# Saltfish-AB/LatentSync

Hardware: AMD Instinct MI355X
Metric: lip-synced frames/sec at 256x256, 16-frame window, 20 DDIM steps (higher is better)
Workload: dtype bf16; 1 GPU; configs[1]: 256x256 x16-frame windows, 20 DDIM steps, guidance 1.0, LatentSync-1.5 UNet + SD-VAE, bf16; 48 independent windows of a clip batched per UNet call; windows_per_rank=240, windows_per_batch=48, frames_per_window=16, global_batch=768, resolution=256, parallelism=dp1 (window sharding, RCCL all-gather of decoded frames)

## Files before the change

include/ls_hip.h:

```cpp
#ifndef LS_HIP_H
#define LS_HIP_H

#include <stddef.h>
#include <stdint.h>

#ifdef __cplusplus
extern "C" {
#endif

#define LS_ABI_VERSION 14

typedef enum {
  LS_OK = 0,
  LS_ERR_INVALID = 1,
  LS_ERR_LAUNCH = 2,
  LS_ERR_WORKSPACE = 3
} ls_status;

enum { LS_ACT_NONE = 0, LS_ACT_GEGLU = 1, LS_ACT_GELU = 2, LS_ACT_SILU = 3 };

typedef struct {
  const uint16_t* x1; const uint16_t* x2;
  int32_t C1, C2;
  int32_t ld1, ld2;
// ... 75 lines not shown
int ls_attention_fp8(const ls_attn_desc* d, void* workspace, size_t workspace_bytes, void* stream);

typedef struct {
  const uint16_t* x;
  int32_t ldx;
  const float* gamma;
  const float* bpe;
  const uint16_t* w;
  uint16_t* o;
  int32_t ldo;
  int32_t C, heads, n_samples, F, S;
  float eps;
} ls_tattn_desc;

int ls_temporal_attention(const ls_tattn_desc* d, void* stream);

typedef struct {
  const void* x;
  const float* ln_rowstats;
  const void* w1;
  const float* b1;
  const void* w2;
  const float* b2;
  void* y;
  int64_t M;
  int32_t ldx, ldy, C, inner;
} ls_ff_desc;

int ls_feedforward(const ls_ff_desc* d, void* stream);

typedef struct {
  const void* o;
  const void* wo;
  const float* bo;
  const void* h1;
  const void* w1;
  const float* b1;
  const void* w2;
  const float* b2;
  const void* wp;
  const float* bp;
  const void* xb;
  void* z;
  float* cs_out;
  int64_t M;
  int32_t ldo, ldh, ldxb, ldz, C, inner;
  float eps;
} ls_ff_chain_desc;

int ls_ff_chain(const ls_ff_chain_desc* d, void* stream);

typedef struct {
  const void* x;
  const float* ln_rowstats;
  const void* wq;
  const float* bq;
  const void* kv;
  const void* wo;
  const float* bo;
  void* y;
  float* stats_out;
  int64_t M;
  int32_t ldx, ldy, ldkv, C, heads, L, hw;
  float eps;
} ls_xattn_desc;

int ls_cross_attention_block(const ls_xattn_desc* d, void* stream);

int ls_small_linear(const float* x, int32_t M, int32_t K, const uint16_t* w, const float* bias, int32_t N,
                    int32_t silu_in, float* y, void* stream);

int ls_timestep_embed(const int32_t* timesteps, const int32_t* step, int32_t B, int32_t dim, int32_t flip,
                      float shift, float* out, void* stream);

int ls_timestep_embed_f32(const float* ts, int32_t B, int32_t dim, int32_t flip, float shift, float* out,
                          void* stream);

int ls_ddim_cfg_step(const uint16_t* eps, int32_t ld_eps, int32_t Bu, int64_t P, float guidance, float* lat,
                     const float* coef, int32_t* step, uint16_t* unet_in, int32_t ld_in, void* stream);

int ls_prep_pixels(const uint8_t* faces, int32_t F, int32_t R, const float* mask, uint16_t* pix, uint16_t* masked,
                   int32_t ld, void* stream);

int ls_vae_sample(const float* moments, int32_t ld_m, const float* eps, int64_t P, float scaling, float shift,
                  uint16_t* dst, int32_t ld_dst, int32_t c_off, void* stream);

int ls_pack_unet_input(const float* lat, const uint16_t* cond, const float* mask, int32_t F, int32_t R, int32_t h,
                       int32_t Bu, uint16_t* unet_in, int32_t ld_in, void* stream);

int ls_scale_latents(const float* lat, int64_t P, float inv_scaling, float shift, uint16_t* z, int32_t ld,
                     void* stream);

int ls_paste_back(const uint16_t* dec, int32_t ld_dec, const uint16_t* pix, int32_t ld_pix, const float* mask,
                  int32_t F, int32_t R, float* out_nchw, uint8_t* out_u8, void* stream);

int ls_add_rows(const uint16_t* x, int64_t rows, int32_t C, int32_t ldx, const float* table, int32_t table_rows,
                uint16_t* y, int32_t ldy, void* stream);

int ls_set_tuning(int32_t key, int32_t value);

int ls_gemm_occupancy(int32_t which);

size_t ls_log_mel_workspace_bytes(int64_t n_samples, int32_t n_mels);
int ls_log_mel(const float* audio, int64_t n_samples, const float* filters, int32_t n_mels, int64_t t_pad,
               uint16_t* out, void* workspace, size_t workspace_bytes, void* stream);

// ... 56 lines not shown
```

latentsync_amd/_lib.py:

```python
import ctypes as C
import os

HERE = os.path.dirname(os.path.abspath(__file__))
LIB_PATH = os.environ.get("LS_HIP_LIB", os.path.join(HERE, "libls_hip.so"))
ABI_VERSION = 14

c_u16p = C.c_void_p
c_vp = C.c_void_p


class ConvDesc(C.Structure):
    _fields_ = [
        ("x1", c_vp), ("x2", c_vp),
        ("C1", C.c_int32), ("C2", C.c_int32),
        ("ld1", C.c_int32), ("ld2", C.c_int32),
        ("n_img", C.c_int32), ("H", C.c_int32), ("W", C.c_int32),
        ("Ho", C.c_int32), ("Wo", C.c_int32),
        ("ksize", C.c_int32), ("stride", C.c_int32), ("pad", C.c_int32), ("upsample", C.c_int32),
        ("aff_scale", c_vp), ("aff_shift", c_vp), ("imgs_per_sample", C.c_int32), ("silu_in", C.c_int32),
        ("w", c_vp), ("K", C.c_int32), ("N", C.c_int32),
        ("bias", c_vp),
        ("rowvec", c_vp), ("rows_per_vec", C.c_int32), ("rowvec_ld", C.c_int32),
        ("res", c_vp), ("ldr", C.c_int32), ("out_scale", C.c_float),
        ("act", C.c_int32),
        ("y", c_vp), ("ldy", C.c_int32), ("y_f32", C.c_int32),
        ("split_k", C.c_int32),
        ("workspace", c_vp), ("workspace_bytes", C.c_size_t),
        ("ln_rowstats", c_vp), ("ln_colsum", c_vp), ("rowvec_mod", C.c_int32),
        ("row_stats_out", c_vp), ("row_stats_eps", C.c_float),
        ("gn_colsum_out", c_vp),
    ]


class ConvPlanInfo(C.Structure):
    _fields_ = [(f, C.c_int32) for f in (
        "family", "bm", "bn", "ks", "tapu", "buf", "epi", "split", "rb_kt", "rb_fm", "rb_flags",
        "halo_bn", "halo_th", "halo_gn", "halo_cs", "halo_ph", "grid", "threads", "lds_bytes",
        "reduce", "colsum_rows", "row_stats")] + [("workspace_bytes", C.c_int64)]


class AttnDesc(C.Structure):
    _fields_ = [("q", c_vp), ("k", c_vp), ("v", c_vp), ("o", c_vp)] + [
        (f"{t}_{s}", C.c_int64) for t in "qkvo" for s in ("sb1", "sb2", "si", "sh")
    ] + [
        ("batch", C.c_int32), ("z2", C.c_int32), ("heads", C.c_int32), ("nq", C.c_int32),
        ("nk", C.c_int32), ("head_dim", C.c_int32), ("scale", C.c_float),
    ]


class TAttnDesc(C.Structure):
    _fields_ = [("x", c_vp), ("ldx", C.c_int32), ("gamma", c_vp), ("bpe", c_vp), ("w", c_vp), ("o", c_vp),
                ("ldo", C.c_int32), ("C", C.c_int32), ("heads", C.c_int32), ("n_samples", C.c_int32),
                ("F", C.c_int32), ("S", C.c_int32), ("eps", C.c_float)]


class FFDesc(C.Structure):
    _fields_ = [("x", c_vp), ("ln_rowstats", c_vp), ("w1", c_vp), ("b1", c_vp), ("w2", c_vp), ("b2", c_vp),
                ("y", c_vp), ("M", C.c_int64), ("ldx", C.c_int32), ("ldy", C.c_int32), ("C", C.c_int32),
                ("inner", C.c_int32)]


class FFChainDesc(C.Structure):
    _fields_ = [("o", c_vp), ("wo", c_vp), ("bo", c_vp), ("h1", c_vp), ("w1", c_vp), ("b1", c_vp), ("w2", c_vp),
                ("b2", c_vp), ("wp", c_vp), ("bp", c_vp), ("xb", c_vp), ("z", c_vp), ("cs_out", c_vp),
                ("M", C.c_int64), ("ldo", C.c_int32), ("ldh", C.c_int32), ("ldxb", C.c_int32), ("ldz", C.c_int32),
                ("C", C.c_int32), ("inner", C.c_int32), ("eps", C.c_float)]


class XAttnDesc(C.Structure):
    _fields_ = [("x", c_vp), ("ln_rowstats", c_vp), ("wq", c_vp), ("bq", c_vp), ("kv", c_vp), ("wo", c_vp),
                ("bo", c_vp), ("y", c_vp), ("stats_out", c_vp), ("M", C.c_int64), ("ldx", C.c_int32),
                ("ldy", C.c_int32), ("ldkv", C.c_int32), ("C", C.c_int32), ("heads", C.c_int32), ("L", C.c_int32),
                ("hw", C.c_int32), ("eps", C.c_float)]


_SIGS = {
    "ls_abi_version": (C.c_int, []),
    "ls_last_error": (C.c_char_p, []),
    "ls_conv2d": (C.c_int, [C.POINTER(ConvDesc), c_vp]),
    "ls_conv_workspace_bytes": (C.c_size_t, [C.POINTER(ConvDesc)]),
    "ls_conv_path": (C.c_int, [C.POINTER(ConvDesc)]),
    "ls_conv_plan": (C.c_int, [C.POINTER(ConvDesc), C.POINTER(ConvPlanInfo)]),
    "ls_groupnorm": (C.c_int, [c_vp, c_vp, C.c_int32, C.c_int32, C.c_int32, C.c_int64, C.c_int32, C.c_float,
                               c_vp, c_vp, c_vp, c_vp, c_vp, C.c_size_t, c_vp]),
    "ls_groupnorm_workspace_bytes": (C.c_size_t, [C.c_int32, C.c_int32]),
    "ls_groupnorm_colsum": (C.c_int, [c_vp, c_vp, C.c_int32, C.c_int32, C.c_int32, C.c_int64, C.c_int32, C.c_float,
                                      c_vp, c_vp, c_vp, c_vp, c_vp]),
    "ls_gn_colsum": (C.c_int, [c_vp, C.c_int64, C.c_int64, C.c_int32, c_vp, c_vp]),
    "ls_groupnorm_apply": (C.c_int, [c_vp, c_vp, C.c_int32, C.c_int32, C.c_int64, C.c_int64, c_vp, c_vp, C.c_int32,
                                     c_vp, c_vp]),
    "ls_layernorm": (C.c_int, [c_vp, C.c_int64, C.c_int64, C.c_int32, C.c_float, c_vp, c_vp, c_vp, C.c_int32, C.c_int32,
                               c_vp, c_vp]),
    "ls_row_stats": (C.c_int, [c_vp, C.c_int64, C.c_int64, C.c_int32, C.c_float, c_vp, c_vp]),
    "ls_attention": (C.c_int, [C.POINTER(AttnDesc), c_vp]),
    "ls_attention_fp8_workspace_bytes": (C.c_size_t, [C.POINTER(AttnDesc)]),
    "ls_attention_fp8": (C.c_int, [C.POINTER(AttnDesc), c_vp, C.c_size_t, c_vp]),
    "ls_temporal_attention": (C.c_int, [C.POINTER(TAttnDesc), c_vp]),
    "ls_feedforward": (C.c_int, [C.POINTER(FFDesc), c_vp]),
    "ls_cross_attention_block": (C.c_int, [C.POINTER(XAttnDesc), c_vp]),
    "ls_ff_chain": (C.c_int, [C.POINTER(FFChainDesc), c_vp]),
    "ls_small_linear": (C.c_int, [c_vp, C.c_int32, C.c_int32, c_vp, c_vp, C.c_int32, C.c_int32, c_vp, c_vp]),
    "ls_timestep_embed": (C.c_int, [c_vp, c_vp, C.c_int32, C.c_int32, C.c_int32, C.c_float, c_vp, c_vp]),
    "ls_timestep_embed_f32": (C.c_int, [c_vp, C.c_int32, C.c_int32, C.c_int32, C.c_float, c_vp, c_vp]),
    "ls_ddim_cfg_step": (C.c_int, [c_vp, C.c_int32, C.c_int32, C.c_int64, C.c_float, c_vp, c_vp, c_vp, c_vp,
                                   C.c_int32, c_vp]),
    "ls_prep_pixels": (C.c_int, [c_vp, C.c_int32, C.c_int32, c_vp, c_vp, c_vp, C.c_int32, c_vp]),
    "ls_vae_sample": (C.c_int, [c_vp, C.c_int32, c_vp, C.c_int64, C.c_float, C.c_float, c_vp, C.c_int32,
                                C.c_int32, c_vp]),
    "ls_pack_unet_input": (C.c_int, [c_vp, c_vp, c_vp, C.c_int32, C.c_int32, C.c_int32, C.c_int32, c_vp,
                                     C.c_int32, c_vp]),
    "ls_scale_latents": (C.c_int, [c_vp, C.c_int64, C.c_float, C.c_float, c_vp, C.c_int32, c_vp]),
    "ls_paste_back": (C.c_int, [c_vp, C.c_int32, c_vp, C.c_int32, c_vp, C.c_int32, C.c_int32, c_vp, c_vp, c_vp]),
    "ls_set_tuning": (C.c_int, [C.c_int32, C.c_int32]),
    "ls_gemm_occupancy": (C.c_int, [C.c_int32]),
    "ls_log_mel_workspace_bytes": (C.c_size_t, [C.c_int64, C.c_int32]),
    "ls_log_mel": (C.c_int, [c_vp, C.c_int64, c_vp, C.c_int32, C.c_int64, c_vp, c_vp, C.c_size_t, c_vp]),
    "ls_resample": (C.c_int, [c_vp, C.c_int64, c_vp, C.c_int32, C.c_int32, C.c_int32, c_vp, C.c_int64, c_vp]),
    "ls_audio_chunks": (C.c_int, [c_vp, C.c_int64, C.c_int32, C.c_int32, C.c_int32, C.c_int32, C.c_double,
                                  C.c_int32, C.c_int32, c_vp, C.c_int32, c_vp]),
    "ls_face_resize_u8": (C.c_int, [c_vp, C.c_int32, C.c_int32, C.c_int32, C.c_int32, C.c_int32, c_vp, c_vp]),
    "ls_resize_faces_u8": (C.c_int, [c_vp, C.c_int32, C.c_int32, C.c_int32, C.c_int32, C.c_int32, c_vp, c_vp]),
    "ls_restore_tables_bytes": (C.c_size_t, [C.c_int32]),
    "ls_restore_init_tables": (C.c_int, [c_vp, C.c_int32, c_vp]),
    "ls_restore_workspace_bytes": (C.c_size_t, [C.c_int32, C.c_int32, C.c_int32]),
    "ls_restore_frames": (C.c_int, [c_vp, C.c_int32, C.c_int32, C.c_int32, c_vp, C.c_int32, C.c_int32, c_vp, c_vp,
                                    C.c_int32, C.c_int32, C.c_int32, c_vp, c_vp, C.c_size_t, c_vp]),
    "ls_resize_lanczos4_workspace_bytes": (C.c_size_t, [C.c_int32, C.c_int32]),
    "ls_resize_lanczos4_u8": (C.c_int, [c_vp, C.c_int32, C.c_int32, C.c_int32, C.c_int32, c_vp, C.c_int32, C.c_int32,
                                        c_vp, C.c_size_t, c_vp]),
    "ls_align_warp_u8": (C.c_int, [c_vp, C.c_int32, C.c_int32, C.c_int32, c_vp, C.c_int32, C.c_int32, C.c_int32,
                                   c_vp, c_vp, c_vp]),
    "ls_mjpeg_restart_interval": (C.c_int, []),
    "ls_mjpeg_workspace_bytes": (C.c_size_t, [C.c_int32, C.c_int32, C.c_int32]),
    "ls_mjpeg_encode": (C.c_int, [c_vp, C.c_int32, C.c_int32, C.c_int32, C.c_int32, c_vp, C.c_int64, c_vp, c_vp,
                                  C.c_size_t, c_vp]),
    "ls_mjpeg_decode_workspace_bytes": (C.c_size_t, [C.c_int32, C.c_int32, C.c_int32]),
    "ls_mjpeg_decode": (C.c_int, [c_vp, C.c_int64, c_vp, C.c_int32, C.c_int32, C.c_int32, c_vp, C.c_int32, c_vp,
                                  C.c_int32, C.c_int32, c_vp, c_vp, c_vp, C.c_size_t, c_vp]),
    "ls_face_brighten_workspace_bytes": (C.c_size_t, [C.c_int32, C.c_int32, C.c_int32, C.c_int32]),
    "ls_face_brighten": (C.c_int, [c_vp, C.c_int32, C.c_int32, C.c_int32, c_vp, c_vp, C.c_int32, C.c_int32, C.c_int32,
                                   C.c_int32, C.c_int32, C.c_int32, c_vp, C.c_int32, C.c_int32, C.c_float, C.c_int32,
                                   C.c_int32, C.c_int32, c_vp, C.c_size_t, c_vp]),
    "ls_add_rows":(C.c_int, [c_vp, C.c_int64, C.c_int32, C.c_int32, c_vp, C.c_int32, c_vp, C.c_int32, c_vp]),
}

EXPORTED = tuple(_SIGS)

_lib = None


def load(path: str = None):
    global _lib
    if _lib is not None:
# ... 22 lines not shown
```

latentsync_amd/build.py:

```python
import concurrent.futures as cf
import os
import re
import shutil
import subprocess
import sys
import tempfile
import warnings

HERE = os.path.dirname(os.path.abspath(__file__))
REPO = os.path.dirname(HERE)
CSRC = os.path.join(HERE, "csrc")
OBJ = os.path.join(REPO, "build", "obj")
LIB = os.path.join(HERE, "libls_hip.so")
HIPCC = os.environ.get("HIPCC", "/opt/rocm/bin/hipcc")
FLAGS = ["--offload-arch=gfx950", "-O3", "-fPIC", "-std=c++17", "-Wno-unused-result", "-munsafe-fp-atomics",
         "-fno-slp-vectorize"]


def _deps():
    hdrs = [os.path.join(CSRC, f) for f in os.listdir(CSRC) if f.endswith(".h")]
    hdrs.append(os.path.join(REPO, "include", "ls_hip.h"))
    return max(os.path.getmtime(h) for h in hdrs)


COUNTED_VMCNT = ("gemm_rowblock_kernel", "conv_gemm_dma_kernel", "attn5_kernel", "attn8_kernel", "tattn_fused_kernel",
                 "attnw_kernel", "conv3x3_halo_kernel", "ff_chain_kernel")


def _spills(stderr):
    bad, cur = [], None
    for line in stderr.splitlines():
        m = re.search(r"remark: +Function Name: (\S+)", line)
        if m:
            cur = m.group(1)
            continue
        m = re.search(r"remark: +VGPRs Spill: (\d+)", line)
        if m and cur and int(m.group(1)) > 0 and any(k in cur for k in COUNTED_VMCNT):
            bad.append(f"{cur}: {line.split('remark:')[1].strip()}")
    return bad


OBJDUMP = os.environ.get("LLVM_OBJDUMP", "/opt/rocm/lib/llvm/bin/llvm-objdump")
_PK_OPSEL = re.compile(r"v_pk_\w+_f32\b[^\n]*\bop_sel:\[([01,]+)\]")


def _packed_opsel(obj):
    skip = os.environ.get("LS_SKIP_OPSEL_GUARD", "") not in ("", "0")
    if not os.path.exists(OBJDUMP):
        if skip:
            warnings.warn(f"packed-fp32 op_sel guard skipped (LS_SKIP_OPSEL_GUARD): {OBJDUMP} not found")
            return []
        raise RuntimeError(f"packed-fp32 op_sel guard: {OBJDUMP} not found (LS_SKIP_OPSEL_GUARD=1 to build without it)")
    with tempfile.TemporaryDirectory() as td:
        cp = os.path.join(td, "k.o")
        shutil.copy(obj, cp)
        r = subprocess.run([OBJDUMP, "--offloading", cp], capture_output=True, text=True, cwd=td)
        dev = [f for f in os.listdir(td) if "gfx950" in f]
        if r.returncode != 0 or not dev:
            msg = f"could not extract the gfx950 code object of {obj} ({r.stderr.strip()[:200]})"
            if skip:
                warnings.warn("packed-fp32 op_sel guard skipped (LS_SKIP_OPSEL_GUARD): " + msg)
                return []
            raise RuntimeError("packed-fp32 op_sel guard: " + msg + " (LS_SKIP_OPSEL_GUARD=1 to build without it)")
        r = subprocess.run([OBJDUMP, "-d", "--mcpu=gfx950", os.path.join(td, dev[0])], capture_output=True, text=True)
    return [m.group(0).split("//")[0].strip() for m in _PK_OPSEL.finditer(r.stdout) if "1" in m.group(1)]


def _compile(src, obj, dep_time):
    if os.path.exists(obj) and os.path.getmtime(obj) >= max(os.path.getmtime(src), dep_time):
        return obj, None
    cmd = [HIPCC] + FLAGS + ["-Rpass-analysis=kernel-resource-usage", "-c", src, "-o", obj]
    r = subprocess.run(cmd, capture_output=True, text=True)
    if r.returncode != 0:
        return obj, r.stderr
    with open(obj[:-2] + ".remarks", "w") as f:
        f.write(r.stderr)
    bad = _spills(r.stderr)
    if bad:
        os.remove(obj)
# ... 38 lines not shown
```

latentsync_amd/ops.py:

```python
import ctypes as C
import math

import torch

from . import _lib
from ._lib import check

ACT_NONE, ACT_GEGLU, ACT_GELU, ACT_SILU = 0, 1, 2, 3
_GN_EPILOGUE = True
GN_SLOT_ROWS = 128
_UPS_PHASE = True


def _p(t):
    return None if t is None else t.data_ptr()


def _stream():
    return torch.cuda.current_stream().cuda_stream


class Workspace:

    def __init__(self, device, gemm_bytes=256 << 20, gn_bytes=24 << 20):
# ... 274 lines not shown
    lib = _lib.load()
    M, C_ = x2d.shape
    if out is None:
        out = torch.empty((M, C_), dtype=torch.bfloat16, device=x2d.device)
    d = _lib.FFDesc()
    d.x, d.ln_rowstats, d.w1, d.b1 = _p(x2d), _p(ln_stats), _p(w1.w), _p(w1.bias)
    d.w2, d.b2, d.y = _p(w2ff), _p(w2.bias), _p(out)
    d.M, d.ldx, d.ldy, d.C, d.inner = M, x2d.stride(0), out.stride(0), C_, w1.N // 2
    check(lib.ls_feedforward(C.byref(d), _stream()), "ls_feedforward")
    return out


class FFChainPack:

    def __init__(self, wo, bo, w1, b1, w2, b2, wp, bp, C, inner, eps):
        self.wo, self.bo, self.w1, self.b1, self.w2, self.b2, self.wp, self.bp = wo, bo, w1, b1, w2, b2, wp, bp
        self.C, self.inner, self.eps = C, inner, eps


def pack_ff_chain(wo: "Packed", ff1: "Packed", ff2: "Packed", po: "Packed", eps=1e-5):
    from .packing import pack_ff_w2, permute_k_acc
    Cc = wo.N
    bf = lambda t: t.to(torch.bfloat16).contiguous()
    w1 = permute_k_acc(ff1.w.float())
    return FFChainPack(bf(pack_ff_w2(wo.w.float()[:, :Cc], permute=False)), wo.bias.float().contiguous(), bf(w1),
                       ff1.bias.float().contiguous(), bf(pack_ff_w2(ff2.w.float()[:, :ff2.K])),
                       ff2.bias.float().contiguous(), bf(pack_ff_w2(po.w.float()[:, :Cc])),
                       po.bias.float().contiguous(), Cc, ff1.N // 2, eps)


def ff_chain_ok(o2d, pk: "FFChainPack"):
    return (pk is not None and o2d.shape[1] == 320 and pk.inner == 1280 and o2d.shape[0] % 128 == 0
            and o2d.stride(1) == 1 and o2d.stride(0) % 8 == 0)


def ff_chain(o2d, h1, xb, pk: "FFChainPack", shape=None, gn_out=True):
    lib = _lib.load()
    M, C_ = o2d.shape
    res = torch.empty(shape or (M, C_), dtype=torch.bfloat16, device=o2d.device)
    out = res.view(M, C_)
    cs = torch.empty((M // GN_SLOT_ROWS, 2, C_), dtype=torch.float32, device=o2d.device) if gn_out else None
    d = _lib.FFChainDesc()
    d.o, d.wo, d.bo, d.h1 = _p(o2d), _p(pk.wo), _p(pk.bo), _p(h1)
    d.w1, d.b1, d.w2, d.b2, d.wp, d.bp = _p(pk.w1), _p(pk.b1), _p(pk.w2), _p(pk.b2), _p(pk.wp), _p(pk.bp)
    d.xb, d.z, d.cs_out = _p(xb), _p(out), _p(cs)
    d.M, d.ldo, d.ldh, d.ldxb, d.ldz = M, o2d.stride(0), h1.stride(0), xb.stride(0), out.stride(0)
    d.C, d.inner, d.eps = C_, pk.inner, float(pk.eps)
    check(lib.ls_ff_chain(C.byref(d), _stream()), "ls_ff_chain")
    if cs is not None:
        res.gn_cs = cs
    return res


class XAttnPack:

    def __init__(self, wq, bq, wo, bo, C, heads):
        self.wq, self.bq, self.wo, self.bo, self.C, self.heads = wq, bq, wo, bo, C, heads


def pack_cross_attention(wq, ln_weight, ln_bias, wo, bo, heads, device):
    from .packing import pack_xattn_q, pack_xattn_wo
    w = wq.float().cpu()
    gamma, beta = ln_weight.float().cpu(), ln_bias.float().cpu()
    pq, pb = pack_xattn_q(w * gamma[None, :], w @ beta, heads)
    po = pack_xattn_wo(wo.float().cpu(), heads)
    bf = lambda t: t.to(torch.bfloat16).to(device).contiguous()
    return XAttnPack(bf(pq), pb.to(device).contiguous(), bf(po), bo.float().to(device).contiguous(), w.shape[0], heads)


def cross_attention_ok(x2d, pk, L, hw):
    return (pk is not None and x2d.shape[1] == 320 and pk.heads == 8 and 1 <= L <= 64 and hw % 128 == 0
            and x2d.shape[0] % hw == 0 and x2d.stride(1) == 1 and x2d.stride(0) % 8 == 0)


def cross_attention_block(x2d, ln_stats, pk: XAttnPack, kv, L, hw, stats_out, out=None, eps=1e-5):
    lib = _lib.load()
    M, C_ = x2d.shape
    if out is None:
        out = torch.empty((M, C_), dtype=torch.bfloat16, device=x2d.device)
    assert stats_out.dtype == torch.float32 and stats_out.is_contiguous() and stats_out.numel() == 2 * M
    assert kv.stride(1) == 1 and kv.shape[0] == (M // hw) * L and kv.shape[1] >= 2 * C_
    d = _lib.XAttnDesc()
    d.x, d.ln_rowstats, d.wq, d.bq, d.kv, d.wo, d.bo = _p(x2d), _p(ln_stats), _p(pk.wq), _p(pk.bq), _p(kv), \
        _p(pk.wo), _p(pk.bo)
    d.y, d.stats_out = _p(out), _p(stats_out)
    d.M, d.ldx, d.ldy, d.ldkv, d.C, d.heads, d.L, d.hw, d.eps = M, x2d.stride(0), out.stride(0), kv.stride(0), C_, \
        pk.heads, L, hw, eps
    check(lib.ls_cross_attention_block(C.byref(d), _stream()), "ls_cross_attention_block")
    return out


def attention_fp8_workspace_bytes(*, batch, heads, nk, head_dim):
    lib = _lib.load()
    d = _lib.AttnDesc()
    d.batch, d.z2, d.heads, d.nq, d.nk, d.head_dim = batch, 1, heads, 1, nk, head_dim
    return lib.ls_attention_fp8_workspace_bytes(C.byref(d))


def small_linear(x, w, bias, silu_in=False, out=None):
    lib = _lib.load()
    M, K = x.shape
    N = w.shape[0]
    if out is None:
        out = torch.empty((M, N), dtype=torch.float32, device=x.device)
    check(lib.ls_small_linear(_p(x), M, K, _p(w), _p(bias), N, int(silu_in), _p(out), _stream()), "ls_small_linear")
    return out
# ... 218 lines not shown
```

latentsync_amd/unet.py:

```python
import math
from dataclasses import dataclass

import torch

from . import ops
from .config import STAGE2_MODEL
from .packing import geglu_interleave, pack_ff_w2, pack_phase_weight, pack_weight, pad_bias
from .schema import unet_param_shapes
from .weights import fill_state_dict

_FUSED_TEMPORAL = True
_FUSED_FF = True
_FF_CHAIN = True
_NARROW_OUT = True
_FUSED_XATTN = False


def _ff(h, st, ff1, ff2, ff2p):
    if ff2p is not None and ops.feedforward_ok(h, ff1, ff2):
        return ops.feedforward(h, st, ff1, ff2, ff2p)
    g = ops.linear(h, ff1, act=ops.ACT_GEGLU, ln_stats=st)
    return ops.linear(g, ff2, res=h)


def _chain_pack(o, ff1, ff2, po, c):
    if not (_FF_CHAIN and _FUSED_FF and c == 320 and ff1.N == 2560 and ff2.N == 320 and ff2.K == 1280):
        return None
    return ops.pack_ff_chain(o, ff1, ff2, po)


def _ff2_packed(dv, key):
    w = dv.sd[key]
    if not _FUSED_FF or tuple(w.shape) != (320, 1280):
        return None
    return pack_ff_w2(w.float().cpu()).to(torch.bfloat16).to(dv.device).contiguous()

_DEFAULTS = dict(
    sample_size=None, in_channels=4, out_channels=4, center_input_sample=False, flip_sin_to_cos=True, freq_shift=0,
    down_block_types=("CrossAttnDownBlock3D", "CrossAttnDownBlock3D", "CrossAttnDownBlock3D", "DownBlock3D"),
    mid_block_type="UNetMidBlock3DCrossAttn",
    up_block_types=("UpBlock3D", "CrossAttnUpBlock3D", "CrossAttnUpBlock3D", "CrossAttnUpBlock3D"),
    only_cross_attention=False, block_out_channels=(320, 640, 1280, 1280), layers_per_block=2, downsample_padding=1,
    mid_block_scale_factor=1, act_fn="silu", norm_num_groups=32, norm_eps=1e-5, cross_attention_dim=1280,
    attention_head_dim=8, dual_cross_attention=False, use_linear_projection=False, class_embed_type=None,
    num_class_embeds=None, upcast_attention=False, resnet_time_scale_shift="default", use_inflated_groupnorm=False,
    use_motion_module=False, motion_module_resolutions=(1, 2, 4, 8), motion_module_mid_block=False,
    motion_module_decoder_only=False, motion_module_type=None, motion_module_kwargs={}, add_audio_layer=False,
)


class FrozenDict(dict):
    def __getattr__(self, k):
        try:
            return self[k]
        except KeyError as e:
            raise AttributeError(k) from e


@dataclass
class UNet3DConditionOutput:
    sample: torch.Tensor

    def __getitem__(self, i):
        return (self.sample,)[i]


def positional_encoding(d_model, max_len=24):
    position = torch.arange(max_len).unsqueeze(1)
# ... 31 lines not shown
            pk.phase = pack_phase_weight(w).to(torch.bfloat16).to(self.device).contiguous()
        return pk

    def packed_ln(self, w, b, ln, geglu=False, pe=None):
        gamma, beta = (t.detach().float().cpu() for t in ln)
        w = w.float().cpu()
        b = (b.float().cpu() if b is not None else torch.zeros(w.shape[0])) + w @ beta
        pk = self.packed(None, w=w * gamma[None, :], b=b, geglu=geglu)
        pk.colsum = pk.w.float().sum(1).contiguous()
        if pe is not None:
            pk.pe_rows = (pe.float().cpu() @ w.T).to(self.device).contiguous()
        return pk


class _Resnet:
    def __init__(self, dv, p, cin, cout, groups, eps, out_scale, temb_slot):
        self.groups, self.eps, self.cin, self.cout = groups, eps, cin, cout
        self.n1 = (dv.f32(p + ".norm1.weight"), dv.f32(p + ".norm1.bias"))
        self.n2 = (dv.f32(p + ".norm2.weight"), dv.f32(p + ".norm2.bias"))
        self.c1 = dv.packed(p + ".conv1.weight", p + ".conv1.bias")
        self.c2 = dv.packed(p + ".conv2.weight", p + ".conv2.bias")
        self.sc = dv.packed(p + ".conv_shortcut.weight", p + ".conv_shortcut.bias") \
            if (p + ".conv_shortcut.weight") in dv.sd else None
        self.out_scale = 1.0 / out_scale
        self.temb_slot = temb_slot

    def __call__(self, x, B, temb_all, x2=None):
        n = x.shape[0]
        F = n // B
        pps = F * x.shape[1] * x.shape[2]
        s1 = ops.group_norm(x, self.groups, self.eps, *self.n1, B, x2=x2)
        rpv = pps * B if temb_all.shape[0] == 1 else pps
        h = ops.conv(x, self.c1, x2=x2, aff=(s1[0], s1[1], F, True), aff_materialize=True,
                     rowvec=(temb_all[:, self.temb_slot:], rpv, temb_all.shape[1]), gn_out=True)
        s2 = ops.group_norm(h, self.groups, self.eps, *self.n2, B)
        res = x if self.sc is None else ops.conv(x, self.sc, x2=x2)
        return ops.conv(h, self.c2, aff=(s2[0], s2[1], F, True), aff_materialize=True, res=res,
                        out_scale=self.out_scale, gn_out=True)


class _Transformer:
    def __init__(self, dv, p, c, heads, groups, audio):
        self.c, self.heads, self.groups = c, heads, groups
        self.fp8 = False
        self.norm = (dv.f32(p + ".norm.weight"), dv.f32(p + ".norm.bias"))
        self.proj_in = dv.packed(p + ".proj_in.weight", p + ".proj_in.bias")
        self.proj_out = dv.packed(p + ".proj_out.weight", p + ".proj_out.bias")
        b = p + ".transformer_blocks.0"
        sd = dv.sd
        ln = lambda k: (sd[k + ".weight"], sd[k + ".bias"])
        self.qkv1 = dv.packed_ln(torch.cat([sd[f"{b}.attn1.to_{n}.weight"] for n in "qkv"], 0), None, ln(b + ".norm1"))
        self.o1 = dv.packed(b + ".attn1.to_out.0.weight", b + ".attn1.to_out.0.bias")
        self.has_audio = audio and (b + ".attn2.to_q.weight") in sd
        if self.has_audio:
            self.q2 = dv.packed_ln(sd[b + ".attn2.to_q.weight"], None, ln(b + ".norm2"))
            self.kv2 = dv.packed(None, w=torch.cat([sd[b + ".attn2.to_k.weight"], sd[b + ".attn2.to_v.weight"]], 0))
            self.o2 = dv.packed(b + ".attn2.to_out.0.weight", b + ".attn2.to_out.0.bias")
            self.xa = ops.pack_cross_attention(
                sd[b + ".attn2.to_q.weight"], *ln(b + ".norm2"), sd[b + ".attn2.to_out.0.weight"],
                sd[b + ".attn2.to_out.0.bias"], heads, dv.device) if _FUSED_XATTN and c == 320 and heads == 8 else None
        self.ff1 = dv.packed_ln(sd[b + ".ff.net.0.proj.weight"], sd[b + ".ff.net.0.proj.bias"], ln(b + ".norm3"),
                                geglu=True)
        self.ff2 = dv.packed(b + ".ff.net.2.weight", b + ".ff.net.2.bias")
        self.ff2p = _ff2_packed(dv, b + ".ff.net.2.weight")
        self.chain = _chain_pack(self.o2, self.ff1, self.ff2, self.proj_out, c) if self.has_audio else None

    def audio_kv(self, audio_rows):
        return ops.linear(audio_rows, self.kv2) if self.has_audio else None

    def __call__(self, x, audio_rows, n_audio_tok, kv=None):
        n, H, W, C = x.shape
        HW = H * W
        rows = n * HW
        d = C // self.heads
        sc = ops.group_norm(x, self.groups, 1e-6, *self.norm, n)
        st = torch.empty((rows, 2), dtype=torch.float32, device=x.device)
        h = ops.conv(x, self.proj_in, aff=(sc[0], sc[1], 1, False), aff_materialize=True,
                     stats_out=st).view(rows, C)
        qkv = ops.linear(h, self.qkv1, ln_stats=st)
        o = torch.empty((rows, C), dtype=torch.bfloat16, device=x.device)
        ops.attention(qkv, qkv[:, C:], qkv[:, 2 * C:], o, batch=n, z2=1, heads=self.heads, nq=HW, nk=HW, head_dim=d,
                      qs=(HW * 3 * C, 0, 3 * C, d), ks=(HW * 3 * C, 0, 3 * C, d), vs=(HW * 3 * C, 0, 3 * C, d),
                      os_=(HW * C, 0, C, d), fp8=self.fp8 and HW > 128 and d in (40, 80))
        h = ops.linear(o, self.o1, res=h, stats_out=st)
        if self.has_audio and audio_rows is not None:
            if kv is None:
                kv = ops.linear(audio_rows, self.kv2)
            L = n_audio_tok
            if ops.cross_attention_ok(h, self.xa, L, HW):
                st2 = torch.empty_like(st)
                h = ops.cross_attention_block(h, st, self.xa, kv, L, HW, st2)
                st = st2
                return self._tail(x, h, st, n, H, W, C)
            q = ops.linear(h, self.q2, ln_stats=st)
            ops.attention(q, kv, kv[:, C:], o, batch=n, z2=1, heads=self.heads, nq=HW, nk=L, head_dim=d,
                          qs=(HW * C, 0, C, d), ks=(L * 2 * C, 0, 2 * C, d), vs=(L * 2 * C, 0, 2 * C, d),
                          os_=(HW * C, 0, C, d))
            if ops.ff_chain_ok(o, self.chain):
                return ops.ff_chain(o, h, x.view(rows, C), self.chain, shape=(n, H, W, C))
            h = ops.linear(o, self.o2, res=h, stats_out=st)
        return self._tail(x, h, st, n, H, W, C)

    def _tail(self, x, h, st, n, H, W, C):
        h = _ff(h, st, self.ff1, self.ff2, self.ff2p)
        return ops.conv(h.view(n, H, W, C), self.proj_out, res=x, gn_out=True)


class _Motion:
    def __init__(self, dv, p, c, heads, groups, kw):
        t = p + ".temporal_transformer"
        b = t + ".transformer_blocks.0"
        sd = dv.sd
        self.c, self.heads, self.groups = c, heads, groups
        self.norm = (dv.f32(t + ".norm.weight"), dv.f32(t + ".norm.bias"))
        self.proj_in = dv.packed(t + ".proj_in.weight", t + ".proj_in.bias")
        self.proj_out = dv.packed(t + ".proj_out.weight", t + ".proj_out.bias")
        self.attn = []
        i = 0
        max_len = kw.get("temporal_position_encoding_max_len", 24)
        while f"{b}.attention_blocks.{i}.to_q.weight" in sd:
            a = f"{b}.attention_blocks.{i}"
            pe = sd.get(a + ".pos_encoder.pe")
            if kw.get("temporal_position_encoding", False):
                pe = (pe.reshape(-1, c) if pe is not None else positional_encoding(c, max_len)).float()
                pe = pe.to(dv.device).contiguous()
            else:
                pe = None
            ln = (sd[f"{b}.norms.{i}.weight"], sd[f"{b}.norms.{i}.bias"])
            wqkv = [sd[f"{a}.to_{n}.weight"] for n in "qkv"]
            self.attn.append(dict(
                qkv=dv.packed_ln(torch.cat(wqkv, 0), None, ln, pe=pe),
                fused=ops.pack_temporal(*wqkv, *ln, pe, heads, dv.device) if c in (320, 640) and heads == 8
                else None,
                o=dv.packed(a + ".to_out.0.weight", a + ".to_out.0.bias")))
            i += 1
        self.ff1 = dv.packed_ln(sd[b + ".ff.net.0.proj.weight"], sd[b + ".ff.net.0.proj.bias"],
                                (sd[b + ".ff_norm.weight"], sd[b + ".ff_norm.bias"]), geglu=True)
        self.ff2 = dv.packed(b + ".ff.net.2.weight", b + ".ff.net.2.bias")
        self.ff2p = _ff2_packed(dv, b + ".ff.net.2.weight")
        self.chain = _chain_pack(self.attn[-1]["o"], self.ff1, self.ff2, self.proj_out, c) if self.attn else None

    def __call__(self, x, B):
        n, H, W, C = x.shape
        F = n // B
        S = H * W
        rows = n * S
        d = C // self.heads
# ... 378 lines not shown
```

Baseline: 158.0 frames/s.

## Fuse back-to-back linears with LayerNorm stats into one chain kernel

Adds a HIP kernel that chains two linears in one launch. The first is either proj_in with the GroupNorm affine applied to the input, or attn1's out-projection with a residual. The kernel computes each row's LayerNorm mean and rstd in-register, normalizes the intermediate, and runs the LN-folded second linear (qkv1 or q2) straight from registers. This removes a kernel launch and the HBM re-read of the intermediate for C=320 transformer blocks. In exchange it is a large hand-tuned kernel with triple-buffered LDS staging, fixed to C=320 and M divisible by 256, and it computes statistics in double.

```diff
diff --git a/include/ls_hip.h b/include/ls_hip.h
--- a/include/ls_hip.h
+++ b/include/ls_hip.h
@@ -151,6 +151,25 @@
 
 typedef struct {
   const void* x;
+  const void* w1;
+  const float* b1;
+  const float* aff_scale;
+  const float* aff_shift;
+  const void* res;
+  const void* w2;
+  const float* b2;
+  void* h;
+  float* stats;
+  void* y;
+  int64_t M, rows_per_sample;
+  int32_t ldx, ldr, ldh, ldy, C, N2;
+  float eps;
+} ls_linear_chain_desc;
+
+int ls_linear_chain(const ls_linear_chain_desc* d, void* stream);
+
+typedef struct {
+  const void* x;
   const float* ln_rowstats;
   const void* wq;
   const float* bq;
diff --git a/latentsync_amd/_lib.py b/latentsync_amd/_lib.py
--- a/latentsync_amd/_lib.py
+++ b/latentsync_amd/_lib.py
@@ -67,6 +67,13 @@
                 ("C", C.c_int32), ("inner", C.c_int32), ("eps", C.c_float)]
 
 
+class LinearChainDesc(C.Structure):
+    _fields_ = [("x", c_vp), ("w1", c_vp), ("b1", c_vp), ("aff_scale", c_vp), ("aff_shift", c_vp), ("res", c_vp),
+                ("w2", c_vp), ("b2", c_vp), ("h", c_vp), ("stats", c_vp), ("y", c_vp), ("M", C.c_int64),
+                ("rows_per_sample", C.c_int64), ("ldx", C.c_int32), ("ldr", C.c_int32), ("ldh", C.c_int32),
+                ("ldy", C.c_int32), ("C", C.c_int32), ("N2", C.c_int32), ("eps", C.c_float)]
+
+
 class XAttnDesc(C.Structure):
     _fields_ = [("x", c_vp), ("ln_rowstats", c_vp), ("wq", c_vp), ("bq", c_vp), ("kv", c_vp), ("wo", c_vp),
                 ("bo", c_vp), ("y", c_vp), ("stats_out", c_vp), ("M", C.c_int64), ("ldx", C.c_int32),
@@ -99,6 +106,7 @@
     "ls_feedforward": (C.c_int, [C.POINTER(FFDesc), c_vp]),
     "ls_cross_attention_block": (C.c_int, [C.POINTER(XAttnDesc), c_vp]),
     "ls_ff_chain": (C.c_int, [C.POINTER(FFChainDesc), c_vp]),
+    "ls_linear_chain": (C.c_int, [C.POINTER(LinearChainDesc), c_vp]),
     "ls_small_linear": (C.c_int, [c_vp, C.c_int32, C.c_int32, c_vp, c_vp, C.c_int32, C.c_int32, c_vp, c_vp]),
     "ls_timestep_embed": (C.c_int, [c_vp, c_vp, C.c_int32, C.c_int32, C.c_int32, C.c_float, c_vp, c_vp]),
     "ls_timestep_embed_f32": (C.c_int, [c_vp, C.c_int32, C.c_int32, C.c_int32, C.c_float, c_vp, c_vp]),
diff --git a/latentsync_amd/build.py b/latentsync_amd/build.py
--- a/latentsync_amd/build.py
+++ b/latentsync_amd/build.py
@@ -24,7 +24,7 @@
 
 
 COUNTED_VMCNT = ("gemm_rowblock_kernel", "conv_gemm_dma_kernel", "attn5_kernel", "attn8_kernel", "tattn_fused_kernel",
-                 "attnw_kernel", "conv3x3_halo_kernel", "ff_chain_kernel")
+                 "attnw_kernel", "conv3x3_halo_kernel", "ff_chain_kernel", "linear_chain_kernel")
 
 
 def _spills(stderr):
diff --git a/latentsync_amd/csrc/ls_chain.hip b/latentsync_amd/csrc/ls_chain.hip
--- /dev/null
+++ b/latentsync_amd/csrc/ls_chain.hip
@@ -0,0 +1,287 @@
+#include "ls_common.h"
+
+namespace ls {
+
+struct ChainArgs {
+  const u16 *x, *w1, *w2, *res;
+  const float *b1, *b2, *aff_scale, *aff_shift;
+  u16 *h, *y;
+  float* stats;
+  int ldx, ldr, ldh, ldy, N2, rps;
+  float eps;
+};
+
+template <int KT, int FM, bool RES>
+__global__ void __launch_bounds__(512) linear_chain_kernel(ChainArgs a) {
+  constexpr int FN = 2, BN = 16 * FN, BM = 8 * 16 * FM, C = 32 * KT;
+  constexpr int KTILES = KT / 2;
+  constexpr int WIMG = BN * KTILES * 8;
+  constexpr int RIMG = RES ? BM * BN / 8 : 0;
+  constexpr int RPT = RIMG / 512;
+  constexpr int STAGE = WIMG + 16 + RIMG;
+  constexpr int PPT = (WIMG + 511) / 512;
+  constexpr int NSTORE = FM * FN;
+  static_assert(KT % 2 == 0 && WIMG % 256 == 0 && RIMG % 512 == 0, "K a multiple of 64");
+  extern __shared__ __attribute__((aligned(16))) uint4 lds_dyn[];
+  const int tid = threadIdx.x, lane = tid & 63, wid = tid >> 6;
+  const int l16 = lane & 15, lg = lane >> 4;
+  const int rb = blockIdx.x;
+  const int mw = rb * BM + wid * 16 * FM;
+  const int nc2 = a.N2 / BN;
+
+  const int wid_u = __builtin_amdgcn_readfirstlane(wid);
+  __builtin_assume(wid_u >= 0 && wid_u < 8);
+  const i32x4 rs_w1 = buffer_rsrc(a.w1, (uint32_t)(C * C * 2));
+  const i32x4 rs_w2 = buffer_rsrc(a.w2, (uint32_t)(a.N2 * C * 2));
+  const i32x4 rs_r = RES ? buffer_rsrc(a.res + (long)rb * BM * a.ldr, (uint32_t)(BM * a.ldr * 2)) : rs_w1;
+  static_assert(8 * BN == 256 && BN / 8 == 4, "piece arithmetic below");
+  int wvo, rvo;
+  {
+    const int t = tid >> 8, row = (tid >> 3) & 31, pc = tid & 7;
+    const int lc = pc ^ ((row >> 1) & 7);
+    wvo = (row * C + t * 64 + lc * 8) * 2;
+    rvo = ((tid >> 2) * a.ldr + (tid & 3) * 8) * 2;
+  }
+  lds_u4* const lbase = (lds_u4*)lds_dyn;
+  auto issue_w = [&](const i32x4& rs, const float* bias, int c, int stage) {
+    lds_u4* const dst = lbase + stage * STAGE;
+#pragma unroll
+    for (int p = 0; p < PPT; ++p) {
+      if (WIMG % 512 == 0 || p * 512 + wid_u * 64 < WIMG)
+        ls_raw_buffer_load_lds(rs, (__attribute__((address_space(3))) void*)(dst + p * 512 + wid_u * 64), 16, wvo,
+                               c * BN * C * 2 + p * 256, 0, 0);
+    }
+    if (wid == 0 && lane < BN / 4) glds16(bias + c * BN + lane * 4, lds_dyn + stage * STAGE + WIMG);
+  };
+  auto issue1 = [&](int c, int stage) {
+    issue_w(rs_w1, a.b1, c, stage);
+    lds_u4* const dst = lbase + stage * STAGE;
+#pragma unroll
+    for (int p = 0; p < RPT; ++p)
+      ls_raw_buffer_load_lds(rs_r, (__attribute__((address_space(3))) void*)(dst + WIMG + 16 + p * 512 + wid_u * 64), 16,
+                             rvo, c * BN * 2 + p * 256 * a.ldr, 0, 0);
+  };
+  auto issue2 = [&](int t, int stage) { issue_w(rs_w2, a.b2, t, stage); };
+
+  issue1(0, 0);
+  bf16x8 ar[FM][KT];
+#pragma unroll
+  for (int i = 0; i < FM; ++i) {
+    const u16* src = a.x + (long)(mw + i * 16 + l16) * a.ldx + lg * 8;
+#pragma unroll
+    for (int s = 0; s < KT; ++s) ar[i][s] = *(const bf16x8*)(src + s * 32);
+  }
+  if (!RES) {
+    const long sb = (long)(mw / a.rps) * C + lg * 8;
+    wait_vm<0>();
+#pragma unroll
+    for (int s = 0; s < KT; ++s) {
+      float sc[8], sh[8];
+      load8f(a.aff_scale + sb + s * 32, sc);
+      load8f(a.aff_shift + sb + s * 32, sh);
+#pragma unroll
+      for (int i = 0; i < FM; ++i) {
+        bf16x8 v = ar[i][s];
+#pragma unroll
+        for (int e = 0; e < 8; ++e) v[e] = (__bf16)fmaf((float)v[e], sc[e], sh[e]);
+        asm volatile("" : "+v"(v));
+        ar[i][s] = v;
+      }
+    }
+  }
+  wait_vm<0>();
+  __builtin_amdgcn_s_barrier();
+  asm volatile("" ::: "memory");
+
+  f32x4 acc[2][FM][FN];
+  bf16x8 op[FM][KT];
+  auto load_prm = [&](int stage, float4 (&bb)[FN]) {
+    const float4* prm = (const float4*)(lds_dyn + stage * STAGE + WIMG);
+#pragma unroll
+    for (int j = 0; j < FN; ++j) bb[j] = prm[lg + 4 * j];
+  };
+  double S1[FM], S2[FM];
+#pragma unroll
+  for (int i = 0; i < FM; ++i) { S1[i] = 0.0; S2[i] = 0.0; }
+  auto epilogue1 = [&](int c, f32x4 (&ac)[FM][FN], int stage) {
+    const int nb = c * BN + 4 * lg;
+    const u16* rtile = (const u16*)(lds_dyn + stage * STAGE + WIMG + 16);
+#pragma unroll
+    for (int i = 0; i < FM; ++i) {
+      u16* hrow = a.h + (long)(mw + i * 16 + l16) * a.ldh;
+      float cs1 = 0.f, cs2 = 0.f;
+      uint2 pk[FN];
+#pragma unroll
+      for (int j = 0; j < FN; ++j) {
+        float r4[4] = {0.f, 0.f, 0.f, 0.f};
+        if (RES) {
+          const uint2 rs = *(const uint2*)(rtile + (wid * 16 * FM + i * 16 + l16) * BN + 4 * lg + 16 * j);
+          r4[0] = __uint_as_float(rs.x << 16); r4[1] = __uint_as_float(rs.x & 0xffff0000u);
+          r4[2] = __uint_as_float(rs.y << 16); r4[3] = __uint_as_float(rs.y & 0xffff0000u);
+        }
+        pk[j] = make_uint2(pack2(ac[i][j][0] + r4[0], ac[i][j][1] + r4[1]), pack2(ac[i][j][2] + r4[2], ac[i][j][3] + r4[3]));
+        *(uint2*)(hrow + nb + 16 * j) = pk[j];
+        typedef __bf16 bf2 __attribute__((ext_vector_type(2)));
+        const bf2 one2 = {(__bf16)1.0f, (__bf16)1.0f};
+        const bf2 px = __builtin_bit_cast(bf2, pk[j].x), py = __builtin_bit_cast(bf2, pk[j].y);
+        cs1 = __builtin_amdgcn_fdot2_f32_bf16(py, one2, __builtin_amdgcn_fdot2_f32_bf16(px, one2, cs1, false), false);
+        cs2 = __builtin_amdgcn_fdot2_f32_bf16(py, py, __builtin_amdgcn_fdot2_f32_bf16(px, px, cs2, false), false);
+      }
+      S1[i] += (double)cs1;
+      S2[i] += (double)cs2;
+      op[i][c] = __builtin_bit_cast(bf16x8, make_uint4(pk[0].x, pk[0].y, pk[1].x, pk[1].y));
+    }
+  };
+  auto epilogue2 = [&](int t, f32x4 (&ac)[FM][FN]) {
+    const int nb = t * BN + 4 * lg;
+#pragma unroll
+    for (int i = 0; i < FM; ++i) {
+      u16* yrow = a.y + (long)(mw + i * 16 + l16) * a.ldy;
+#pragma unroll
+      for (int j = 0; j < FN; ++j)
+        *(uint2*)(yrow + nb + 16 * j) = make_uint2(pack2(ac[i][j][0], ac[i][j][1]), pack2(ac[i][j][2], ac[i][j][3]));
+    }
+  };
+  auto mfma_chunk = [&](const bf16x8 (&b)[FM][KT], int stage, f32x4 (&ac)[FM][FN], const float4 (&b0)[FN]) {
+    const uint4* cur = lds_dyn + stage * STAGE;
+#pragma unroll
+    for (int i = 0; i < FM; ++i)
+#pragma unroll
+      for (int j = 0; j < FN; ++j) ac[i][j] = (f32x4){b0[j].x, b0[j].y, b0[j].z, b0[j].w};
+#pragma unroll
+    for (int s = 0; s < KT; ++s) {
+      bf16x8 bw[FN];
+      const int ch = (s & 1) * 4 + lg;
+#pragma unroll
+      for (int j = 0; j < FN; ++j)
+        bw[j] = __builtin_bit_cast(bf16x8, cur[(s >> 1) * (8 * BN) + swz64(j * 16 + l16, ch)]);
+#pragma unroll
+      for (int i = 0; i < FM; ++i)
+#pragma unroll
+        for (int j = 0; j < FN; ++j)
+          ac[i][j] = __builtin_amdgcn_mfma_f32_16x16x32_bf16(bw[j], b[i][s], ac[i][j], 0, 0, 0);
+    }
+  };
+  auto sync = [&]() {
+    asm volatile("s_waitcnt lgkmcnt(0)" ::: "memory");
+    __builtin_amdgcn_s_barrier();
+    asm volatile("" ::: "memory");
+  };
+
+  {
+    float4 bn[FN];
+    load_prm(0, bn);
+    issue1(1, 1);
+    mfma_chunk(ar, 0, acc[0], bn);
+  }
+  wait_vm<0>();
+  sync();
+#pragma unroll
+  for (int c = 1; c < KT; ++c) {
+    float4 bn[FN];
+    load_prm(c % 3, bn);
+    if (c + 1 < KT) issue1(c + 1, (c + 1) % 3);
+    else issue2(0, (c + 1) % 3);
+    mfma_chunk(ar, c % 3, acc[c & 1], bn);
+    epilogue1(c - 1, acc[(c - 1) & 1], (c - 1) % 3);
+    wait_vm<NSTORE>();
+    sync();
+  }
+  epilogue1(KT - 1, acc[(KT - 1) & 1], (KT - 1) % 3);
+
+#pragma unroll
+  for (int i = 0; i < FM; ++i) {
+    double s1 = S1[i], s2 = S2[i];
+#pragma unroll
+    for (int o = 16; o < 64; o <<= 1) {
+      s1 += __shfl_xor(s1, o, 64);
+      s2 += __shfl_xor(s2, o, 64);
+    }
+    const double n = (double)C, mean = s1 / n;
+    const double var = fmax(s2 / n - mean * mean, 0.0);
+    const float meanf = (float)mean, rstd = (float)(1.0 / sqrt(var + (double)a.eps));
+    if (lg == 0) *(float2*)(a.stats + 2L * (mw + i * 16 + l16)) = make_float2(meanf, rstd);
+    const float nmr = -meanf * rstd;
+#pragma unroll
+    for (int s = 0; s < KT; ++s) {
+      bf16x8 v = op[i][s];
+#pragma unroll
+      for (int e = 0; e < 8; ++e) v[e] = (__bf16)fmaf((float)v[e], rstd, nmr);
+      op[i][s] = v;
+    }
+  }
+
+  {
+    float4 bn[FN];
+    load_prm(KT % 3, bn);
+    issue2(min(1, nc2 - 1), (KT + 1) % 3);
+    mfma_chunk(op, KT % 3, acc[0], bn);
+  }
+  wait_vm<0>();
+  sync();
+  auto body2 = [&](int t, f32x4 (&ac)[FM][FN], f32x4 (&prev)[FM][FN]) {
+    const int st = (KT + t) % 3;
+    float4 bn[FN];
+    load_prm(st, bn);
+    issue2(min(t + 1, nc2 - 1), st == 2 ? 0 : st + 1);
+    mfma_chunk(op, st, ac, bn);
+    epilogue2(t - 1, prev);
+    wait_vm<NSTORE>();
+    sync();
+  };
+  int t = 1;
+  for (; t + 1 < nc2; t += 2) {
+    body2(t, acc[1], acc[0]);
+    body2(t + 1, acc[0], acc[1]);
+  }
+  if (t < nc2) {
+    body2(t, acc[1], acc[0]);
+    epilogue2(t, acc[1]);
+  } else {
+    epilogue2(nc2 - 1, acc[0]);
+  }
+}
+
+template <int KT, int FM, bool RES>
+static int launch_chain(const ChainArgs& a, long M, hipStream_t s) {
+  constexpr int BM = 128 * FM;
+  constexpr size_t shm = (size_t)3 * (32 * (KT / 2) * 8 + 16 + (RES ? BM * 32 / 8 : 0)) * 16;
+  LS_SET_MAX_DYN_SHM((linear_chain_kernel<KT, FM, RES>), (int)shm);
+  linear_chain_kernel<KT, FM, RES><<<(unsigned)(M / BM), 512, shm, s>>>(a);
+  return check_launch("linear_chain_kernel");
+}
+
+}
+
+using namespace ls;
+
+extern "C" int ls_linear_chain(const ls_linear_chain_desc* d, void* stream) {
+  if (!d || !d->x || !d->w1 || !d->b1 || !d->w2 || !d->b2 || !d->h || !d->stats || !d->y)
+    return fail(LS_ERR_INVALID, "ls_linear_chain: null pointer");
+  const bool aff = d->aff_scale || d->aff_shift;
+  if (aff == (d->res != nullptr) || (aff && (!d->aff_scale || !d->aff_shift)))
+    return fail(LS_ERR_INVALID, "ls_linear_chain: either aff_scale + aff_shift (form i) or res (form ii)");
+  if (d->C != 320) return fail(LS_ERR_INVALID, "ls_linear_chain: C = 320 only");
+  if (d->N2 != d->C && d->N2 != 3 * d->C) return fail(LS_ERR_INVALID, "ls_linear_chain: N2 = C or 3 C only");
+  const int bm = 256;
+  if (d->M <= 0 || d->M % bm || d->M > 0x7fffffffL)
+    return fail(LS_ERR_INVALID, "ls_linear_chain: M a positive multiple of 256, < 2^31");
+  const int32_t ldmax = 1 << 20;
+  if (d->ldx < d->C || d->ldh < d->C || d->ldy < d->N2 || d->ldx % 8 || d->ldh % 4 || d->ldy % 4 || d->ldx > ldmax ||
+      d->ldh > ldmax || d->ldy > ldmax || (d->res && (d->ldr < d->C || d->ldr % 8 || d->ldr > ldmax)))
+    return fail(LS_ERR_INVALID, "ls_linear_chain: pitches >= the row length, <= 2^20 (x, res: % 8; h, y: % 4)");
+  if (aff && (d->rows_per_sample <= 0 || d->rows_per_sample > 0x7fffffffL || d->rows_per_sample % (bm / 8)))
+    return fail(LS_ERR_INVALID, "ls_linear_chain: rows_per_sample a positive multiple of 32 (a wave's rows)");
+  if ((((uintptr_t)d->x | (uintptr_t)d->w1 | (uintptr_t)d->w2 | (uintptr_t)d->b1 | (uintptr_t)d->b2 | (uintptr_t)d->res |
+        (uintptr_t)d->aff_scale | (uintptr_t)d->aff_shift) & 15) ||
+      (((uintptr_t)d->h | (uintptr_t)d->y | (uintptr_t)d->stats) & 7))
+    return fail(LS_ERR_INVALID, "ls_linear_chain: x / w1 / w2 / b1 / b2 / res / aff 16-B aligned, h / y / stats 8-B aligned");
+  ChainArgs a;
+  a.x = (const u16*)d->x; a.w1 = (const u16*)d->w1; a.w2 = (const u16*)d->w2; a.res = (const u16*)d->res;
+  a.b1 = d->b1; a.b2 = d->b2; a.aff_scale = d->aff_scale; a.aff_shift = d->aff_shift;
+  a.h = (u16*)d->h; a.y = (u16*)d->y; a.stats = d->stats;
+  a.ldx = d->ldx; a.ldr = d->ldr; a.ldh = d->ldh; a.ldy = d->ldy; a.N2 = d->N2; a.rps = (int)d->rows_per_sample;
+  a.eps = d->eps;
+  hipStream_t s = (hipStream_t)stream;
+  return aff ? launch_chain<10, 2, false>(a, d->M, s) : launch_chain<10, 2, true>(a, d->M, s);
+}
diff --git a/latentsync_amd/ops.py b/latentsync_amd/ops.py
--- a/latentsync_amd/ops.py
+++ b/latentsync_amd/ops.py
@@ -350,6 +350,51 @@
     return res
 
 
+class LinearChainPack:
+
+    def __init__(self, w1, b1, w2, b2, C, N2, eps):
+        self.w1, self.b1, self.w2, self.b2, self.C, self.N2, self.eps = w1, b1, w2, b2, C, N2, eps
+
+
+def pack_linear_chain(first: "Packed", second_ln: "Packed", eps=1e-5):
+    from .packing import permute_k_acc
+    assert second_ln.colsum is not None, "the second linear must be LayerNorm-folded"
+    w2 = permute_k_acc(second_ln.w.float()).to(torch.bfloat16).contiguous()
+    return LinearChainPack(first.w, first.bias, w2, second_ln.bias.float().contiguous(), first.N, second_ln.N, eps)
+
+
+def linear_chain_ok(x2d, pk: "LinearChainPack", *, res=None, rows_per_sample=None):
+    if pk is None or pk.C != 320 or tuple(pk.w1.shape) != (pk.C, pk.C) or pk.N2 not in (pk.C, 3 * pk.C):
+        return False
+    bm = 256
+    if x2d.dim() != 2 or x2d.shape[1] != pk.C or x2d.shape[0] % bm or x2d.stride(1) != 1 or x2d.stride(0) % 8:
+        return False
+    if res is not None:
+        return res.stride(1) == 1 and res.stride(0) % 8 == 0 and res.data_ptr() % 16 == 0
+    return rows_per_sample is not None and rows_per_sample % (bm // 8) == 0
+
+
+def linear_chain(x2d, pk: "LinearChainPack", stats_out, *, aff=None, rows_per_sample=0, res=None, h=None, out=None):
+    lib = _lib.load()
+    M, C_ = x2d.shape
+    if h is None:
+        h = torch.empty((M, C_), dtype=torch.bfloat16, device=x2d.device)
+    if out is None:
+        out = torch.empty((M, pk.N2), dtype=torch.bfloat16, device=x2d.device)
+    assert stats_out.dtype == torch.float32 and stats_out.is_contiguous() and stats_out.numel() == 2 * M
+    assert tuple(h.shape) == (M, C_) and tuple(out.shape) == (M, pk.N2)
+    d = _lib.LinearChainDesc()
+    d.x, d.w1, d.b1, d.w2, d.b2 = _p(x2d), _p(pk.w1), _p(pk.b1), _p(pk.w2), _p(pk.b2)
+    if aff is not None:
+        d.aff_scale, d.aff_shift, d.rows_per_sample = _p(aff[0]), _p(aff[1]), rows_per_sample
+    if res is not None:
+        d.res, d.ldr = _p(res), res.stride(0)
+    d.h, d.stats, d.y = _p(h), _p(stats_out), _p(out)
+    d.M, d.ldx, d.ldh, d.ldy, d.C, d.N2, d.eps = M, x2d.stride(0), h.stride(0), out.stride(0), C_, pk.N2, float(pk.eps)
+    check(lib.ls_linear_chain(C.byref(d), _stream()), "ls_linear_chain")
+    return h, out
+
+
 class XAttnPack:
 
     def __init__(self, wq, bq, wo, bo, C, heads):
diff --git a/latentsync_amd/unet.py b/latentsync_amd/unet.py
--- a/latentsync_amd/unet.py
+++ b/latentsync_amd/unet.py
@@ -14,6 +14,7 @@
 _FF_CHAIN = True
 _NARROW_OUT = True
 _FUSED_XATTN = False
+_LINEAR_CHAIN = frozenset({("B", 320), ("A", 320)})
 
 
 def _ff(h, st, ff1, ff2, ff2p):
@@ -151,8 +152,12 @@
         self.qkv1 = dv.packed_ln(torch.cat([sd[f"{b}.attn1.to_{n}.weight"] for n in "qkv"], 0), None, ln(b + ".norm1"))
         self.o1 = dv.packed(b + ".attn1.to_out.0.weight", b + ".attn1.to_out.0.bias")
         self.has_audio = audio and (b + ".attn2.to_q.weight") in sd
+        self.chain_b = ops.pack_linear_chain(self.proj_in, self.qkv1) if ("B", c) in _LINEAR_CHAIN else None
+        self.chain_a = None
         if self.has_audio:
             self.q2 = dv.packed_ln(sd[b + ".attn2.to_q.weight"], None, ln(b + ".norm2"))
+            if ("A", c) in _LINEAR_CHAIN:
+                self.chain_a = ops.pack_linear_chain(self.o1, self.q2)
             self.kv2 = dv.packed(None, w=torch.cat([sd[b + ".attn2.to_k.weight"], sd[b + ".attn2.to_v.weight"]], 0))
             self.o2 = dv.packed(b + ".attn2.to_out.0.weight", b + ".attn2.to_out.0.bias")
             self.xa = ops.pack_cross_attention(
@@ -174,15 +179,24 @@
         d = C // self.heads
         sc = ops.group_norm(x, self.groups, 1e-6, *self.norm, n)
         st = torch.empty((rows, 2), dtype=torch.float32, device=x.device)
-        h = ops.conv(x, self.proj_in, aff=(sc[0], sc[1], 1, False), aff_materialize=True,
-                     stats_out=st).view(rows, C)
-        qkv = ops.linear(h, self.qkv1, ln_stats=st)
+        if ops.linear_chain_ok(x.view(rows, C), self.chain_b, rows_per_sample=HW):
+            h, qkv = ops.linear_chain(x.view(rows, C), self.chain_b, st, aff=(sc[0], sc[1]), rows_per_sample=HW)
+        else:
+            h = ops.conv(x, self.proj_in, aff=(sc[0], sc[1], 1, False), aff_materialize=True,
+                         stats_out=st).view(rows, C)
+            qkv = ops.linear(h, self.qkv1, ln_stats=st)
         o = torch.empty((rows, C), dtype=torch.bfloat16, device=x.device)
         ops.attention(qkv, qkv[:, C:], qkv[:, 2 * C:], o, batch=n, z2=1, heads=self.heads, nq=HW, nk=HW, head_dim=d,
                       qs=(HW * 3 * C, 0, 3 * C, d), ks=(HW * 3 * C, 0, 3 * C, d), vs=(HW * 3 * C, 0, 3 * C, d),
                       os_=(HW * C, 0, C, d), fp8=self.fp8 and HW > 128 and d in (40, 80))
-        h = ops.linear(o, self.o1, res=h, stats_out=st)
-        if self.has_audio and audio_rows is not None:
+        audio = self.has_audio and audio_rows is not None
+        q = None
+        if audio and not ops.cross_attention_ok(h, self.xa, n_audio_tok, HW) and \
+                ops.linear_chain_ok(o, self.chain_a, res=h):
+            h, q = ops.linear_chain(o, self.chain_a, st, res=h)
+        else:
+            h = ops.linear(o, self.o1, res=h, stats_out=st)
+        if audio:
             if kv is None:
                 kv = ops.linear(audio_rows, self.kv2)
             L = n_audio_tok
@@ -191,7 +205,8 @@
                 h = ops.cross_attention_block(h, st, self.xa, kv, L, HW, st2)
                 st = st2
                 return self._tail(x, h, st, n, H, W, C)
-            q = ops.linear(h, self.q2, ln_stats=st)
+            if q is None:
+                q = ops.linear(h, self.q2, ln_stats=st)
             ops.attention(q, kv, kv[:, C:], o, batch=n, z2=1, heads=self.heads, nq=HW, nk=L, head_dim=d,
                           qs=(HW * C, 0, C, d), ks=(L * 2 * C, 0, 2 * C, d), vs=(L * 2 * C, 0, 2 * C, d),
                           os_=(HW * C, 0, C, d))
```

Result: no change. 158.5 frames/s, median of 6 (+0.3%).
